# KaffinPX/neptune-core

Measured on AMD Instinct MI355X. Metric: STARK proofs verified/sec (whole node) + Tip5 perms/sec vs VALU roofline, higher is better.
Workload: dtype u64 (Goldilocks mod p; XFE = cubic extension)

## Files before the change

neptune-core_amd/csrc/stark_kernels.hip:

```cpp
#include <hip/hip_ext.h>

#include <atomic>
#include <cstdlib>

#include "../../include/nhip_challenge_id.h"
#include "kernels.hpp"
#include "proof_codec.hpp"
#include "stark.hpp"
#include "tip5_device.hpp"
#include "xfe.hpp"

namespace nhip {

#ifndef NHIP_LAT_PRIO
#define NHIP_LAT_PRIO 2
#endif
__device__ __forceinline__ void latency_priority() {
    if constexpr (NHIP_LAT_PRIO > 0) __builtin_amdgcn_s_setprio(NHIP_LAT_PRIO);
}
static constexpr uint32_t AGE_PRIO_OLDEST = 2;
static constexpr uint32_t AGE_PRIO_MIN_PROOFS = 2048;
__device__ uint32_t g_batches_done;
struct AgePrio {
    uint32_t seq, k;
};
__device__ __forceinline__ void age_priority(AgePrio a, int base) {
    bool old = false;
    if (a.k) {
        const uint32_t done = __builtin_amdgcn_readfirstlane(
            __hip_atomic_load(&g_batches_done, __ATOMIC_RELAXED, __HIP_MEMORY_SCOPE_AGENT));
        old = (int32_t)(a.seq - done) < (int32_t)a.k;
    }
    switch (base + (old ? 1 : 0)) {
        case 0: break;
        case 1: __builtin_amdgcn_s_setprio(1); break;
        case 2: __builtin_amdgcn_s_setprio(2); break;
        default: __builtin_amdgcn_s_setprio(3); break;
    }
}
#ifndef NHIP_MP_PRIO
#define NHIP_MP_PRIO 1
#endif


template <bool MW>
__device__ __forceinline__ Xfe ld_xfe_w(const uint64_t* __restrict__ w, uint64_t off) {
    return {word_mont<MW>(w[off]), word_mont<MW>(w[off + 1]), word_mont<MW>(w[off + 2])};
}
__device__ __forceinline__ Xfe ld_xfe_raw(const uint64_t* __restrict__ w, uint64_t off) {
    return {w[off], w[off + 1], w[off + 2]};
}
__device__ __forceinline__ void st_xfe_raw(uint64_t* __restrict__ w, uint64_t off, Xfe v) {
    w[off] = v.c0;
    w[off + 1] = v.c1;
    w[off + 2] = v.c2;
}
__device__ __forceinline__ bool x_is_zero(Xfe a) { return (a.c0 | a.c1 | a.c2) == 0; }

__device__ __forceinline__ uint64_t root_of_unity(uint32_t log2n) {
    return b_pow(to_mont(7), (GL_P - 1) >> log2n);
}

template <bool MW>
__global__ void __launch_bounds__(64) k_decode(const uint64_t* __restrict__ words, const ProofIn* __restrict__ in,
                                               uint32_t n_proofs, Dims D, uint32_t fs_stride, uint32_t xs_stride,
                                               ProofDesc* __restrict__ desc, FsOp* __restrict__ ops,
                                               uint32_t* __restrict__ fail, unsigned long long* __restrict__ counters) {
    latency_priority();
    __shared__ ProofDesc spd;
    __shared__ uint32_t sfail;
    __shared__ int sdeg;
    const uint32_t p = blockIdx.x, lane = threadIdx.x;
    if (p >= n_proofs) return;
    const ProofIn pin = in[p];
    if (lane == 0) {
        uint64_t perms = 0, perms_lcw = 0;
        const ClaimLoc cl{pin.claim_off, pin.claim_in_n, pin.claim_out_n};
        uint32_t f = decode_stream<MW>(words, pin.off, pin.len, cl, D, spd, ops + (uint64_t)p * fs_stride, perms, perms_lcw);
        if (!f && spd.log2_ph != pin.sized_log2_ph) {
            f = FAIL_DECODE;
            spd = ProofDesc{};
            claim_offsets(spd, cl);
        }
        if (!f) {
            atomicAdd(counters + CNT_PERMS_STATIC, (unsigned long long)perms);
            atomicAdd(counters + CNT_PERMS_LCW, (unsigned long long)perms_lcw);
        }
        sfail = f;
        sdeg = -1;
    }
    __syncthreads();
    const uint32_t f = sfail;
    if (!f) {
        int deg = -1;
        for (uint32_t hi = spd.last_poly_n; hi > 0; hi = hi > 64 ? hi - 64 : 0) {
            bool nz = false;
            if (lane < hi) {
                const uint64_t* x = words + spd.last_poly_off + 3ull * (hi - 1 - lane);
                nz = (canon(x[0]) | canon(x[1]) | canon(x[2])) != 0;
            }
            const uint64_t b = __ballot(nz);
            if (b) {
                deg = (int)(hi - (uint32_t)__ffsll((unsigned long long)b));
                break;
            }
        }
        if (lane == 0) sdeg = deg;
    }
    __syncthreads();
    if (lane == 0) {
        if (!f) last_poly_finish(spd, sdeg, D);
        const SampleLayout sl = SampleLayout::of(D.d, spd.R);
        spd.fs_op_off = p * fs_stride;
        spd.xs_off = (uint64_t)p * xs_stride;
        spd.n_xs = f ? 0u : sl.total;
        spd.idx_off = (uint64_t)p * D.d.num_checks;
        fail[p] = f;
    }
    __syncthreads();
    const uint64_t* src = reinterpret_cast<const uint64_t*>(&spd);
    uint64_t* dst = reinterpret_cast<uint64_t*>(desc + p);
    for (uint32_t i = lane; i < sizeof(ProofDesc) / 8; i += 64) dst[i] = src[i];
}

template <bool PAIR, bool MW>
__device__ __forceinline__ void fs_replay_wide_body(uint32_t bx, const Tip5Lds& lds, const uint64_t* __restrict__ words,
                                                    const ProofDesc* __restrict__ desc,
                                                    const FsOp* __restrict__ ops, uint32_t n_proofs,
                                                    uint64_t* __restrict__ xs, uint32_t* __restrict__ idx_out,
                                                    const uint32_t* __restrict__ fail) {
    constexpr uint32_t LANES = PAIR ? 32u : 16u;
    const uint32_t e = threadIdx.x & 15u;
    const uint32_t h = PAIR ? (threadIdx.x >> 4) & 1u : 0u;
    const uint32_t g = (bx * blockDim.x + threadIdx.x) / LANES;
    if (g >= n_proofs || fail[g]) return;
    uint64_t rc[TIP5_ROUNDS];
#pragma unroll
    for (int r = 0; r < TIP5_ROUNDS; ++r) rc[r] = c_tip5_rc_raw[r * 16 + e];
    uint32_t cm[8];
#pragma unroll
    for (int j = 0; j < 8; ++j) cm[j] = h ? TIP5_MDS[j + 8] : TIP5_MDS[j];
    auto permute = [&](uint64_t st) {
        if constexpr (PAIR) return tip5_permute_pair(st, e, h, rc, cm, lds.lut);
        else return tip5_permute_wide<false>(st, e, rc, lds.lut);
    };
    const bool writer = h == 0;
    const ProofDesc& d = desc[g];
    uint64_t s = 0;
    uint64_t xcur = d.xs_off * 3;
    uint64_t icur = d.idx_off;
    const uint32_t row_shift = threadIdx.x & (64u - LANES);
    for (uint32_t o = 0; o < d.fs_op_n; ++o) {
        const FsOp op = ops[d.fs_op_off + o];
        if (op.kind == FS_ABSORB) {
            const uint64_t* __restrict__ src = words + op.arg;
            const uint32_t len = op.n;
            const uint32_t nchunks = len / TIP5_RATE + 1;
            uint64_t w = (e < TIP5_RATE && e < len) ? src[e] : 0ull;
            for (uint32_t c = 0; c < nchunks; ++c) {
                const uint32_t pos = c * TIP5_RATE;
                const uint64_t cur = w;
                const uint32_t ni = pos + TIP5_RATE + e;
                w = (e < TIP5_RATE && ni < len) ? src[ni] : 0ull;
                if (e < TIP5_RATE) {
                    const uint32_t rem = len - pos;
                    s = e < rem ? word_mont<MW>(cur) : (e == rem ? MONT_ONE : 0ull);
                }
                s = permute(s);
            }
        } else if (op.kind == FS_SQUEEZE_X) {
            const uint32_t nwords = 3 * op.n;
            for (uint32_t f = 0; f < nwords; f += TIP5_RATE) {
                if (writer && e < TIP5_RATE && f + e < nwords) xs[xcur + f + e] = s;
                s = permute(s);
            }
            xcur += nwords;
        } else {
            const uint64_t bound = op.arg;
            uint32_t got = 0;
            while (got < op.n) {
                const uint64_t v = from_mont(s);
                s = permute(s);
                const bool valid = e < TIP5_RATE && v != GL_P - 1;
                const uint64_t ball = __ballot(valid);
                const uint32_t bits = (uint32_t)(ball >> row_shift) & 0x3FFu;
                const uint32_t rank = __popc(bits & ((1u << e) - 1u));
                if (writer && valid && got + rank < op.n) idx_out[icur + got + rank] = (uint32_t)((v & 0xFFFFFFFFull) % bound);
                got += __popc(bits);
            }
            icur += op.n;
        }
    }
}
template <bool PAIR, bool MW>
__global__ void __launch_bounds__(256) k_fs_replay_wide(const uint64_t* __restrict__ words,
                                                        const ProofDesc* __restrict__ desc,
                                                        const FsOp* __restrict__ ops, uint32_t n_proofs,
                                                        uint64_t* __restrict__ xs, uint32_t* __restrict__ idx_out,
                                                        const uint32_t* __restrict__ fail, AgePrio age) {
    age_priority(age, NHIP_LAT_PRIO);
    __shared__ Tip5Lds lds;
    tip5_lds_init(lds);
    fs_replay_wide_body<PAIR, MW>(blockIdx.x, lds, words, desc, ops, n_proofs, xs, idx_out, fail);
}

#ifndef NHIP_QUAD_PRIO
#define NHIP_QUAD_PRIO NHIP_LAT_PRIO
#endif
template <bool MW>
__global__ void __launch_bounds__(1024) k_fs_replay_quad(const uint64_t* __restrict__ words,
                                                       const ProofDesc* __restrict__ desc,
                                                       const FsOp* __restrict__ ops, uint32_t n_proofs,
                                                       uint64_t* __restrict__ xs, uint32_t* __restrict__ idx_out,
// ... 732 lines not shown
        __syncthreads();
    }
}

template <bool MW>
__device__ __forceinline__ void mp_roots_body(uint32_t i, const uint64_t* __restrict__ words,
                                              const ProofDesc* __restrict__ desc, const uint64_t* __restrict__ dig,
                                              MpPlan plan, uint32_t n_records, uint32_t trees_per_proof, uint32_t k,
                                              uint32_t* __restrict__ fail, uint32_t n_proofs, LcwTree lcw) {
    if (i >= n_records) {
        const uint32_t p = i - n_records;
        if (p >= n_proofs || (fail[p] & FAIL_DECODE)) return;
        const ProofDesc& d = desc[p];
        uint64_t v[5];
        lcw_node<MW>(words, d, lcw.nodes + (uint64_t)p * lcw.max_len * 5, 1, d.last_cw_n, v);
        bool ok = true;
#pragma unroll
        for (int q = 0; q < 5; ++q) ok &= v[q] == word_mont<MW>(words[d.fri_root[d.R] + q]);
        if (!ok) atomicOr(&fail[p], FAIL_FRI_LAST_ROOT);
        return;
    }
    const MpRoot r = plan.roots[i];
    if (r.code == MPS_NONE) return;
    const uint32_t p = i / trees_per_proof, tree = i - p * trees_per_proof;
    const ProofDesc& d = desc[p];
    const uint64_t grp_id = (uint64_t)p * (trees_per_proof - 3) + (tree < 4 ? 0u : tree - 3);
    const uint32_t nd = plan.ndup[grp_id];
    bool ok = true;
    for (uint32_t j = 0; j < nd; ++j) {
        uint64_t a[5], b[5];
        mp_load<MW>(mp_leaf_code(d, p, tree, k, plan.dups[(grp_id * k + j) * 2]), words, dig, nullptr, a);
        mp_load<MW>(mp_leaf_code(d, p, tree, k, plan.dups[(grp_id * k + j) * 2 + 1]), words, dig, nullptr, b);
#pragma unroll
        for (int q = 0; q < 5; ++q) ok &= a[q] == b[q];
    }
    uint64_t v[5];
    mp_load<MW>(r.code, words, dig, plan.arena, v);
#pragma unroll
    for (int q = 0; q < 5; ++q) ok &= v[q] == word_mont<MW>(words[r.root_off + q]);
    if (!ok) atomicOr(&fail[p], r.fail_bit);
}
template <bool MW>
__global__ void k_mp_roots(const uint64_t* __restrict__ words, const ProofDesc* __restrict__ desc,
                           const uint64_t* __restrict__ dig, MpPlan plan, uint32_t n_records, uint32_t trees_per_proof,
                           uint32_t k, uint32_t* __restrict__ fail, uint32_t n_proofs, LcwTree lcw) {
    mp_roots_body<MW>(blockIdx.x * blockDim.x + threadIdx.x, words, desc, dig, plan, n_records, trees_per_proof, k,
                      fail, n_proofs, lcw);
}

__device__ Xfe block_sum_xfe(Xfe v, Xfe* sh) {
    const uint32_t tid = threadIdx.x;
    sh[tid] = v;
    __syncthreads();
    for (uint32_t s = blockDim.x >> 1; s > 0; s >>= 1) {
        if (tid < s) sh[tid] = x_add(sh[tid], sh[tid + s]);
        __syncthreads();
    }
    const Xfe r = sh[0];
    __syncthreads();
    return r;
}

__device__ __forceinline__ Xfe shfl_xor_xfe_fwd(Xfe v, int m) {
    return {(uint64_t)__shfl_xor((long long)v.c0, m), (uint64_t)__shfl_xor((long long)v.c1, m),
            (uint64_t)__shfl_xor((long long)v.c2, m)};
}

__device__ Xfe block_sum_xfe_waves(Xfe v, Xfe* sh) {
    const uint32_t tid = threadIdx.x, nw = blockDim.x >> 6;
#pragma unroll
    for (int m = 32; m > 0; m >>= 1) v = x_add(v, shfl_xor_xfe_fwd(v, m));
    if ((tid & 63u) == 0) sh[tid >> 6] = v;
    __syncthreads();
    Xfe r = sh[0];
    for (uint32_t w = 1; w < nw; ++w) r = x_add(r, sh[w]);
    __syncthreads();
    return r;
}

static constexpr uint32_t CH_COMPRESS_PROGRAM_DIGEST = NHIP_CH_CompressProgramDigestIndeterminate,
                          CH_STANDARD_INPUT = NHIP_CH_StandardInputIndeterminate,
                          CH_STANDARD_OUTPUT = NHIP_CH_StandardOutputIndeterminate,
                          CH_LOOKUP_TABLE_PUBLIC = NHIP_CH_LookupTablePublicIndeterminate;
static_assert(CH_LOOKUP_TABLE_PUBLIC == 54 && NHIP_CHALLENGE_SAMPLE_COUNT == 59 && NHIP_CHALLENGE_COUNT == 63,
              "triton-air ChallengeId layout");
static_assert(NHIP_CH_StandardInputTerminal == NHIP_CHALLENGE_SAMPLE_COUNT && NHIP_CH_CompressedProgramDigest == 62,
              "derived challenges follow the sampled ones");

__device__ __forceinline__ Xfe shfl_xor_xfe(Xfe v, int m) {
    return {(uint64_t)__shfl_xor((long long)v.c0, m), (uint64_t)__shfl_xor((long long)v.c1, m),
            (uint64_t)__shfl_xor((long long)v.c2, m)};
}

template <class Sym>
__device__ Xfe eval_terminal_wave(uint32_t n, Xfe c, Sym sym) {
    const uint32_t lane = threadIdx.x & 63u;
    uint32_t s = 0;
    while (s < 6u && (1u << s) < n + 1u) ++s;
    const uint32_t L = 1u << s, ch = (n + L) >> s, pad = L * ch - n;
    auto entry = [&](uint32_t pos) -> Xfe {
        if (lane >= L) return x_zero();
        if (pos >= pad) return x_lift(sym(pos - pad));
        return pos + 1u == pad ? x_one() : x_zero();
    };
    Xfe h = entry(lane * ch), m = c;
    for (uint32_t k = 1; k < ch; ++k) {
        h = x_add(x_mul(h, c), entry(lane * ch + k));
        m = x_mul(m, c);
    }
    for (uint32_t k = 0; k < s; ++k) {
        const Xfe o = shfl_xor_xfe(h, 1 << k);
        const bool up = (lane >> k) & 1u;
        h = x_add(x_mul(up ? o : h, m), up ? h : o);
        if (k + 1u < s) m = x_mul(m, m);
    }
    return h;
}

#ifndef NHIP_OOD_WAVES
#define NHIP_OOD_WAVES 1
#endif

template <uint32_t BLOCK, bool MW, bool GS>
__global__ void __launch_bounds__(BLOCK, BLOCK == 256 ? NHIP_OOD_WAVES : 1) k_ood_air(const uint64_t* __restrict__ words, const ProofDesc* __restrict__ desc,
                                                 uint32_t n_proofs, StarkDims dims, const OodIns* __restrict__ prog,
                                                 const uint32_t* __restrict__ seg_off, uint32_t n_levels,
                                                 const Xfe* __restrict__ consts, uint4 cons_type_off,
                                                 const uint64_t* __restrict__ xs, uint64_t* __restrict__ ood_out,
                                                 uint32_t* __restrict__ fail, uint32_t lds_slots,
                                                 Xfe* __restrict__ gslots, uint32_t gslot_n) {
    latency_priority();
    extern __shared__ __attribute__((aligned(16))) unsigned char smem[];
    Xfe* red = reinterpret_cast<Xfe*>(smem);
    Xfe* zinv = red + 16;
    Xfe* chal_derived = zinv + 4;
    Xfe* misc = chal_derived + 4;
    uint32_t& zero_flag = *reinterpret_cast<uint32_t*>(misc + 4);
    Xfe* val = reinterpret_cast<Xfe*>(smem + AIR_LDS_HEADER);
    const uint32_t p = blockIdx.x, tid = threadIdx.x;
    Xfe* gval = gslots + (uint64_t)p * gslot_n;
    auto slot_ld = [&](uint32_t s) -> Xfe { return !GS || s < lds_slots ? val[s] : gval[s - lds_slots]; };
    auto slot_st = [&](uint32_t s, const Xfe& v) {
        if (!GS || s < lds_slots) val[s] = v;
        else gval[s - lds_slots] = v;
    };
    if (p >= n_proofs || (fail[p] & FAIL_DECODE)) return;
    const ProofDesc& d = desc[p];
    const SampleLayout sl = SampleLayout::of(dims, d.R);
    const uint64_t xb = d.xs_off * 3;
    const Xfe z = ld_xfe_raw(xs, xb + 3ull * sl.z);
    if (tid == 0) zero_flag = 0;
    __syncthreads();
    if (tid == 0) {
        const uint64_t w_inv = b_inv(root_of_unity(d.log2_ph));
        const Xfe except_last = x_sub(z, x_lift(w_inv));
        const Xfe zm1 = x_sub(z, x_one());
        Xfe zph = z;
        for (uint32_t q = 0; q < d.log2_ph; ++q) zph = x_mul(zph, zph);
        const Xfe cons = x_sub(zph, x_one());
        const bool z0 = x_is_zero(zm1), z1 = x_is_zero(cons), z3 = x_is_zero(except_last);
        if (z0 || z1 || z3) zero_flag = 1u;
        const Xfe a = z0 ? x_one() : zm1, b = z1 ? x_one() : cons, c = z3 ? x_one() : except_last;
        const Xfe ab = x_mul(a, b);
        const Xfe iabc = x_inv(x_mul(ab, c));
        const Xfe iab = x_mul(iabc, c);
        const Xfe i1 = z1 ? x_zero() : x_mul(iab, a);
        zinv[0] = z0 ? x_zero() : x_mul(iab, b);
        zinv[1] = i1;
        zinv[2] = x_mul(except_last, i1);
        zinv[3] = z3 ? x_zero() : x_mul(iabc, ab);
    } else if (tid >= 64 && tid < 256) {
        auto chal = [&](uint32_t i) { return ld_xfe_raw(xs, xb + 3ull * (sl.chal + i)); };
        const uint32_t wv = tid >> 6;
        if (wv == 1) {
            const Xfe lut = eval_terminal_wave(256u, chal(CH_LOOKUP_TABLE_PUBLIC), [&](uint32_t i) {
                const uint64_t y = i + 1;
                return to_mont((y * y % 257u * y % 257u + 256u) % 257u);
            });
            if (tid == 64) chal_derived[2] = lut;
        } else if (wv == 2) {
            const Xfe ein = eval_terminal_wave(d.claim_in_n, chal(CH_STANDARD_INPUT),
                                               [&](uint32_t i) { return word_mont<MW>(words[d.claim_in_off + i]); });
            const Xfe comp = eval_terminal_wave(5u, chal(CH_COMPRESS_PROGRAM_DIGEST),
                                                [&](uint32_t i) { return word_mont<MW>(words[d.claim_digest_off + i]); });
            if (tid == 128) {
                chal_derived[0] = ein;
                chal_derived[3] = comp;
            }
        } else {
            const Xfe eout = eval_terminal_wave(d.claim_out_n, chal(CH_STANDARD_OUTPUT),
                                                [&](uint32_t i) { return word_mont<MW>(words[d.claim_out_off + i]); });
            if (tid == 192) chal_derived[1] = eout;
        }
    }
    __syncthreads();
    const uint32_t offs[5] = {0u, cons_type_off.x, cons_type_off.y, cons_type_off.z, cons_type_off.w};
    auto fetch = [&](uint32_t ref) -> Xfe {
        const uint32_t t = ref >> 30;
        if (t == 0) return slot_ld(ref);
        if (t == 1) return consts[ref & 0x3FFFFFFFu];
        const uint32_t kind = (ref >> 27) & 7u, i = ref & 0x7FFFFFFu;
        switch (kind) {
            case IN_MAIN_CURR: return ld_xfe_w<MW>(words, d.ood_mc + 3ull * i);
            case IN_AUX_CURR: return ld_xfe_w<MW>(words, d.ood_ac + 3ull * i);
            case IN_MAIN_NEXT: return ld_xfe_w<MW>(words, d.ood_mn + 3ull * i);
            case IN_AUX_NEXT: return ld_xfe_w<MW>(words, d.ood_an + 3ull * i);
            default:
                return i < dims.num_sampled ? ld_xfe_raw(xs, xb + 3ull * (sl.chal + i)) : chal_derived[i - dims.num_sampled];
        }
    };
    for (uint32_t lvl = 0; lvl < n_levels; ++lvl) {
        const uint32_t s0 = seg_off[3 * lvl], s1 = seg_off[3 * lvl + 1], s2 = seg_off[3 * lvl + 2],
                       s3 = seg_off[3 * lvl + 3];
        for (uint32_t q = s0 + tid; q < s1; q += blockDim.x) {
            const uint4 ins = reinterpret_cast<const uint4*>(prog)[q];
            slot_st(ins.w, fetch(ins.y));
        }
        for (uint32_t q = s1 + tid; q < s2; q += blockDim.x) {
            const uint4 ins = reinterpret_cast<const uint4*>(prog)[q];
            slot_st(ins.w, x_mul(slot_ld(ins.y), slot_ld(ins.z)));
        }
        for (uint32_t q = s2 + tid; q < s3; q += blockDim.x) {
            const uint4 ins = reinterpret_cast<const uint4*>(prog)[q];
            const Xfe x = slot_ld(ins.y), y = slot_ld(ins.z);
            slot_st(ins.w, ins.x == OOD_ADD ? x_add(x, y) : x_sub(x, y));
        }
        __syncthreads();
    }
    const uint32_t C = dims.num_constraints, cbase = lds_slots + gslot_n - C;
    Xfe acc = x_zero();
    for (uint32_t c = tid; c < C; c += blockDim.x) {
        uint32_t t = 0;
        while (t < 3 && c >= offs[t + 1]) ++t;
        const Xfe w = ld_xfe_raw(xs, xb + 3ull * (sl.quot_w + c));
        acc = x_add(acc, x_mul(w, x_mul(slot_ld(cbase + c), zinv[t])));
    }
    const Xfe ood_q = block_sum_xfe_waves(acc, red);
    const uint32_t M = dims.num_main, A = dims.num_aux, Q = dims.num_quot_seg;
    Xfe lc = x_zero(), ln = x_zero();
    for (uint32_t c = tid; c < M + A; c += blockDim.x) {
        const Xfe w = ld_xfe_raw(xs, xb + 3ull * (sl.lin_w + c));
        const Xfe vc = c < M ? ld_xfe_w<MW>(words, d.ood_mc + 3ull * c) : ld_xfe_w<MW>(words, d.ood_ac + 3ull * (c - M));
        const Xfe vn = c < M ? ld_xfe_w<MW>(words, d.ood_mn + 3ull * c) : ld_xfe_w<MW>(words, d.ood_an + 3ull * (c - M));
        lc = x_add(lc, x_mul(w, vc));
        ln = x_add(ln, x_mul(w, vn));
    }
    const Xfe sum_c = block_sum_xfe_waves(lc, red);
    const Xfe sum_n = block_sum_xfe_waves(ln, red);
    if (tid >= 64) return;
    Xfe seg = x_zero(), qlin = x_zero();
    for (uint32_t base = 0; base < Q; base += 64u) {
        const uint32_t q = base + tid, top = min(Q - 1u, base + 63u);
        Xfe zk = (q & 1u) ? z : x_one(), zp = z;
        for (uint32_t e = top >> 1, bit = 1; e; e >>= 1, ++bit) {
            zp = x_mul(zp, zp);
            zk = x_mul(zk, ((q >> bit) & 1u) ? zp : x_one());
        }
        if (q < Q) {
            const Xfe sq = ld_xfe_w<MW>(words, d.ood_qs + 3ull * q);
            seg = x_add(seg, x_mul(zk, sq));
            qlin = x_add(qlin, x_mul(ld_xfe_raw(xs, xb + 3ull * (sl.lin_w + M + A + q)), sq));
        }
    }
#pragma unroll
    for (int m = 32; m > 0; m >>= 1) {
        seg = x_add(seg, shfl_xor_xfe(seg, m));
        qlin = x_add(qlin, shfl_xor_xfe(qlin, m));
    }
    if (tid == 0) {
        uint32_t f = 0;
        if (zero_flag) f |= FAIL_ZERO_INVERSE;
        if (!x_eq(seg, ood_q)) f |= FAIL_OOD;
        if (f) atomicOr(&fail[p], f);
        uint64_t* o = ood_out + (uint64_t)p * 9;
        st_xfe_raw(o, 0, sum_c);
        st_xfe_raw(o, 3, sum_n);
        st_xfe_raw(o, 6, qlin);
    }
}

__device__ __forceinline__ uint64_t lds_pow(const uint64_t* __restrict__ sq, uint64_t e) {
    uint64_t r = MONT_ONE;
    for (uint32_t b = 0; e; ++b, e >>= 1)
        if (e & 1) r = mont_mul(r, sq[b]);
    return r;
}

#ifndef NHIP_FRI_WAVES
#define NHIP_FRI_WAVES 1
#endif
template <bool MW>
__device__ __forceinline__ void fri_body(uint32_t p, const uint64_t* __restrict__ words, const ProofDesc* __restrict__ desc,
                                         uint32_t n_proofs, StarkDims dims, const uint64_t* __restrict__ xs,
                                         const uint32_t* __restrict__ idx_all, uint64_t* __restrict__ xdom,
                                         uint32_t* __restrict__ fail) {
    __shared__ Xfe red[256];
    __shared__ uint64_t gsq[33], wsq[33];
    __shared__ uint32_t lflag;
    const uint32_t tid = threadIdx.x;
    if (p >= n_proofs || (fail[p] & FAIL_DECODE)) return;
    const ProofDesc& d = desc[p];
    const SampleLayout sl = SampleLayout::of(dims, d.R);
    const uint64_t xb = d.xs_off * 3;
    const uint32_t k = dims.num_checks;
    const uint32_t* __restrict__ idx = idx_all + d.idx_off;
    const uint32_t L = d.last_cw_n;
    const uint32_t log2L = 31 - __clz(L);
    if (tid == 0) {
        lflag = 0;
        uint64_t g = root_of_unity(d.log2_N);
        for (uint32_t q = 0; q < d.log2_N; ++q, g = mont_mul(g, g)) gsq[q] = g;
    } else if (tid == 64) {
        uint64_t w = root_of_unity(log2L);
        for (uint32_t q = 0; q < log2L; ++q, w = mont_mul(w, w)) wsq[q] = w;
    }
    __syncthreads();
    uint32_t f = 0;
    if (tid < k) {
        const uint32_t i0 = idx[tid];
        Xfe a = ld_xfe_w<MW>(words, d.fri[0].leaves_off + 3ull * tid);
        uint64_t x = mont_mul(to_mont(7), lds_pow(gsq, i0));
        xdom[(uint64_t)p * k + tid] = x;
        uint64_t xinv = b_inv(x);
        const uint64_t neg_half = to_mont((GL_P - 1) / 2);
        for (uint32_t r = 0; r < d.R; ++r) {
            const Xfe b = ld_xfe_w<MW>(words, d.fri[1 + r].leaves_off + 3ull * tid);
            const Xfe alpha = ld_xfe_raw(xs, xb + 3ull * (sl.alpha + r));
            const Xfe slope = x_scale(x_sub(b, a), mont_mul(neg_half, xinv));
            a = x_add(a, x_mul(slope, x_sub(alpha, x_lift(x))));
            x = mont_mul(x, x);
            xinv = mont_mul(xinv, xinv);
        }
        const Xfe last = ld_xfe_w<MW>(words, d.last_cw_off + 3ull * (i0 & (L - 1)));
        if (!x_eq(last, a)) f |= FAIL_FRI_LAST_AGREE;
    }
    const Xfe t = ld_xfe_raw(xs, xb + 3ull * sl.indeterminate);
    Xfe num = x_zero(), den = x_zero();
    if (tid < L) {
        uint64_t wi = lds_pow(wsq, tid);
        const uint64_t wstep = blockDim.x < L ? wsq[31 - __clz(blockDim.x)] : MONT_ONE;
        auto term = [&](uint32_t i, uint64_t w, Xfe inv) {
            const Xfe q = x_scale(inv, w);
            num = x_add(num, x_mul(q, ld_xfe_w<MW>(words, d.last_cw_off + 3ull * i)));
            den = x_add(den, q);
        };
        uint32_t i = tid;
        for (; i + blockDim.x < L; i += 2 * blockDim.x) {
            const uint64_t w1 = mont_mul(wi, wstep);
            const Xfe d0 = x_sub(t, x_lift(wi)), d1 = x_sub(t, x_lift(w1));
            const Xfe pr = x_mul(d0, d1);
            if (x_is_zero(pr)) {
                atomicOr(&lflag, 1u);
                term(i, wi, x_inv(d0));
                term(i + blockDim.x, w1, x_inv(d1));
            } else {
                const Xfe inv = x_inv(pr);
                term(i, wi, x_mul(inv, d1));
                term(i + blockDim.x, w1, x_mul(inv, d0));
            }
            wi = mont_mul(w1, wstep);
        }
        if (i < L) {
            const Xfe diff = x_sub(t, x_lift(wi));
            if (x_is_zero(diff)) atomicOr(&lflag, 1u);
            term(i, wi, x_inv(diff));
        }
    }
    const Xfe snum = block_sum_xfe(num, red);
    const Xfe sden = block_sum_xfe(den, red);
    __shared__ Xfe tpow[32];
    const uint32_t pbits = d.last_poly_n ? 32 - __clz(d.last_poly_n) : 0;
    if (tid == 0) {
        Xfe q = t;
        for (uint32_t j = 0; j < pbits; ++j, q = x_mul(q, q)) tpow[j] = q;
    }
    __syncthreads();
    Xfe hp = x_zero();
    for (uint32_t c = tid; c < d.last_poly_n; c += blockDim.x) {
        Xfe pw = x_one();
        for (uint32_t j = 0; (c >> j) != 0; ++j)
            if ((c >> j) & 1u) pw = x_mul(pw, tpow[j]);
        hp = x_add(hp, x_mul(pw, ld_xfe_w<MW>(words, d.last_poly_off + 3ull * c)));
    }
    const Xfe h = block_sum_xfe(hp, red);
    if (tid == 0) {
        if (lflag || x_is_zero(sden)) f |= FAIL_ZERO_INVERSE;
        else if (!x_eq(h, x_mul(snum, x_inv(sden)))) f |= FAIL_FRI_EVAL;
        if (!d.last_poly_degree_ok) f |= FAIL_FRI_DEGREE;
    }
    if (f) atomicOr(&fail[p], f);
}
template <bool MW>
__global__ void __launch_bounds__(256, NHIP_FRI_WAVES) k_fri(const uint64_t* __restrict__ words, const ProofDesc* __restrict__ desc,
                                             uint32_t n_proofs, StarkDims dims, const uint64_t* __restrict__ xs,
                                             const uint32_t* __restrict__ idx_all, uint64_t* __restrict__ xdom,
                                             uint32_t* __restrict__ fail) {
    latency_priority();
    fri_body<MW>(blockIdx.x, words, desc, n_proofs, dims, xs, idx_all, xdom, fail);
}

template <bool MW>
__global__ void __launch_bounds__(256) k_plan_fri_small(const uint64_t* __restrict__ words,
                                                        const ProofDesc* __restrict__ desc, uint32_t n_proofs,
                                                        uint32_t k, uint32_t trees_per_proof, uint32_t groups,
                                                        const uint64_t* __restrict__ dig,
                                                        const uint32_t* __restrict__ idx_all, MpPlan plan,
                                                        uint32_t* __restrict__ fail,
                                                        unsigned long long* __restrict__ perm_counter,
                                                        StarkDims dims, const uint64_t* __restrict__ xs,
                                                        uint64_t* __restrict__ xdom) {
    latency_priority();
    const uint32_t bx = blockIdx.x, np = n_proofs * groups;
    if (bx < np)
        mp_plan_body<256>(bx % n_proofs, bx / n_proofs, words, desc, n_proofs, k, trees_per_proof, dig, idx_all, plan,
                          fail, perm_counter);
    else
        fri_body<MW>(bx - np, words, desc, n_proofs, dims, xs, idx_all, xdom, fail);
}

typedef unsigned __int128 u128_t;
static constexpr uint32_t DEEP_UNROLL = 8;

__device__ __forceinline__ uint64_t reduce_u108(u128_t y) {
    const uint64_t y0 = (uint64_t)y, y1 = (uint64_t)(y >> 64);
    const uint64_t r = reduce96(y0, (uint32_t)y1);
    return gl_sub(r, y1 >> 32);
}

__device__ __forceinline__ uint64_t shfl_xor_u64(uint64_t v, int m) {
    return (uint64_t)__shfl_xor((long long)v, m);
}

__device__ __forceinline__ uint4 w_limbs(uint64_t w) {
    return make_uint4((uint32_t)w & 0x3FFFFFu, (uint32_t)(w >> 22) & 0x3FFFFFu, (uint32_t)(w >> 44), 0u);
}
__device__ __forceinline__ void wl_mac(uint64_t (&a)[6], uint4 wl, uint32_t x0, uint32_t x1) {
    a[0] += (uint64_t)wl.x * x0;
    a[1] += (uint64_t)wl.y * x0;
    a[2] += (uint64_t)wl.z * x0;
    a[3] += (uint64_t)wl.x * x1;
    a[4] += (uint64_t)wl.y * x1;
    a[5] += (uint64_t)wl.z * x1;
}
__device__ __forceinline__ uint64_t wl_reduce(const uint64_t (&a)[6]) {
    const u128_t U = (u128_t)a[0] + ((u128_t)a[1] << 22) + ((u128_t)a[2] << 44);
    const u128_t W = (u128_t)a[3] + ((u128_t)a[4] << 22) + ((u128_t)a[5] << 44);
    const uint64_t ur = reduce_u108(U), wr = reduce_u108(W);
    return gl_add(ur, reduce96(wr << 32, (uint32_t)(wr >> 32)));
}

#ifndef NHIP_DEEP_WAVES
#define NHIP_DEEP_WAVES 6
#endif
template <bool MW>
__global__ void __launch_bounds__(256, NHIP_DEEP_WAVES) k_deep_rows8(const uint64_t* __restrict__ words,
                                                    const ProofDesc* __restrict__ desc, uint32_t n_proofs,
                                                    StarkDims dims, const uint64_t* __restrict__ xs,
                                                    const uint64_t* __restrict__ xdom,
                                                    const uint64_t* __restrict__ ood, uint32_t* __restrict__ fail) {
    extern __shared__ __attribute__((aligned(16))) unsigned char smem[];
    const uint32_t M = dims.num_main, A = dims.num_aux, Q = dims.num_quot_seg, k = dims.num_checks;
    uint4* wm = reinterpret_cast<uint4*>(smem);
    uint4* wa = wm + 3 * M;
    Xfe* rowsum = reinterpret_cast<Xfe*>(wa + 9 * A);
    __shared__ Xfe s_quot[MAX_CHECKS];
    __shared__ Xfe s_at[3];
    const uint32_t p = blockIdx.x, tid = threadIdx.x;
    if (p >= n_proofs || (fail[p] & FAIL_DECODE)) return;
    const ProofDesc& d = desc[p];
    const SampleLayout sl = SampleLayout::of(dims, d.R);
    const uint64_t xb = d.xs_off * 3;
    const uint64_t* __restrict__ lw = xs + xb + 3ull * sl.lin_w;
    for (uint32_t i = tid; i < 3 * M; i += blockDim.x) wm[i] = w_limbs(lw[i]);
    for (uint32_t c = tid; c < A; c += blockDim.x) {
        const uint64_t w0 = lw[3 * (M + c)], w1 = lw[3 * (M + c) + 1], w2 = lw[3 * (M + c) + 2];
        uint4* o = wa + 9 * c;
        o[0] = w_limbs(w0), o[1] = w_limbs(w1), o[2] = w_limbs(w2);
        o[3] = w_limbs(gl_sub(0, w2)), o[4] = w_limbs(gl_add(w0, w2)), o[5] = w_limbs(w1);
        o[6] = w_limbs(gl_sub(0, w1)), o[7] = w_limbs(gl_sub(w1, w2)), o[8] = w_limbs(gl_add(w0, w2));
    }
    if (tid == blockDim.x - 1) {
        const Xfe z = ld_xfe_raw(xs, xb + 3ull * sl.z);
        s_at[0] = z;
        s_at[1] = x_scale(z, root_of_unity(d.log2_ph));
        Xfe zq = x_one();
        for (uint32_t q = 0; q < Q; ++q) zq = x_mul(zq, z);
        s_at[2] = zq;
    }
    __syncthreads();
    const uint32_t q8 = tid & 7u, rloc = tid >> 3;
    const uint32_t rows_per_pass = blockDim.x >> 3;
    for (uint32_t j0 = 0; j0 < k; j0 += rows_per_pass) {
        const uint32_t j = j0 + rloc;
        uint64_t acc[3][6];
#pragma unroll
        for (int c = 0; c < 3; ++c)
#pragma unroll
            for (int q = 0; q < 6; ++q) acc[c][q] = 0;
        if (j < k) {
            const uint64_t* __restrict__ mrow = words + d.main_rows_off + (uint64_t)j * M;
            uint32_t c = q8;
            for (; c + 8 * (DEEP_UNROLL - 1) < M; c += 8 * DEEP_UNROLL) {
                uint64_t xv[DEEP_UNROLL];
#pragma unroll
                for (uint32_t u = 0; u < DEEP_UNROLL; ++u) xv[u] = mrow[c + 8 * u];
#pragma unroll
                for (uint32_t u = 0; u < DEEP_UNROLL; ++u) {
                    const uint32_t cc = c + 8 * u, x0 = (uint32_t)xv[u], x1 = (uint32_t)(xv[u] >> 32);
                    wl_mac(acc[0], wm[3 * cc], x0, x1);
                    wl_mac(acc[1], wm[3 * cc + 1], x0, x1);
                    wl_mac(acc[2], wm[3 * cc + 2], x0, x1);
                }
            }
            for (; c < M; c += 8) {
                const uint64_t xw = mrow[c];
                const uint32_t x0 = (uint32_t)xw, x1 = (uint32_t)(xw >> 32);
                wl_mac(acc[0], wm[3 * c], x0, x1);
                wl_mac(acc[1], wm[3 * c + 1], x0, x1);
                wl_mac(acc[2], wm[3 * c + 2], x0, x1);
            }
            const uint64_t* __restrict__ arow = words + d.aux_rows_off + (uint64_t)j * 3 * A;
            const uint32_t WA = 3 * A;
            uint32_t w = q8;
            for (; w + 8 * (DEEP_UNROLL - 1) < WA; w += 8 * DEEP_UNROLL) {
                uint64_t xv[DEEP_UNROLL];
#pragma unroll
                for (uint32_t u = 0; u < DEEP_UNROLL; ++u) xv[u] = arow[w + 8 * u];
#pragma unroll
                for (uint32_t u = 0; u < DEEP_UNROLL; ++u) {
                    const uint4* wt = wa + 3 * (w + 8 * u);
                    const uint32_t x0 = (uint32_t)xv[u], x1 = (uint32_t)(xv[u] >> 32);
                    wl_mac(acc[0], wt[0], x0, x1);
                    wl_mac(acc[1], wt[1], x0, x1);
                    wl_mac(acc[2], wt[2], x0, x1);
                }
            }
            for (; w < WA; w += 8) {
                const uint4* wt = wa + 3 * w;
                const uint64_t xw = arow[w];
                const uint32_t x0 = (uint32_t)xw, x1 = (uint32_t)(xw >> 32);
                wl_mac(acc[0], wt[0], x0, x1);
                wl_mac(acc[1], wt[1], x0, x1);
                wl_mac(acc[2], wt[2], x0, x1);
            }
        }
        uint64_t v0 = wl_reduce(acc[0]), v1 = wl_reduce(acc[1]), v2 = wl_reduce(acc[2]);
#pragma unroll
        for (int m = 1; m < 8; m <<= 1) {
            v0 = gl_add(v0, shfl_xor_u64(v0, m));
            v1 = gl_add(v1, shfl_xor_u64(v1, m));
            v2 = gl_add(v2, shfl_xor_u64(v2, m));
        }
        if (j < k && q8 == 0) {
            if constexpr (MW) rowsum[j] = {from_mont(v0), from_mont(v1), from_mont(v2)};
            else rowsum[j] = {v0, v1, v2};
        }
        if (j < k && q8 == 1) {
            Xfe qv = x_zero();
            for (uint32_t q = 0; q < Q; ++q)
                qv = x_add(qv, x_mul(ld_xfe_raw(lw, 3ull * (M + A + q)),
                                     ld_xfe_raw(words, d.quot_rows_off + (uint64_t)j * 3 * Q + 3ull * q)));
            if constexpr (MW) s_quot[j] = qv;
            else s_quot[j] = {to_mont(qv.c0), to_mont(qv.c1), to_mont(qv.c2)};
        }
    }
    __syncthreads();
    uint32_t f = 0;
    for (uint32_t j2 = tid; j2 < k; j2 += blockDim.x) {
        const Xfe row = rowsum[j2];
        const Xfe x = x_lift(xdom[(uint64_t)p * k + j2]);
        const Xfe d0 = x_sub(x, s_at[0]), d1 = x_sub(x, s_at[1]), d2 = x_sub(x, s_at[2]);
        const Xfe d01 = x_mul(d0, d1);
        const Xfe prod = x_mul(d01, d2);
        if (x_is_zero(prod)) {
            f |= FAIL_ZERO_INVERSE;
            continue;
        }
        const Xfe inv = x_inv(prod);
        const Xfe inv2 = x_mul(inv, d01);
        const Xfe inv01 = x_mul(inv, d2);
        const Xfe inv0 = x_mul(inv01, d1);
        const Xfe inv1 = x_mul(inv01, d0);
        const uint64_t* __restrict__ oo = ood + (uint64_t)p * 9;
        const uint64_t* __restrict__ wd = lw + 3ull * (M + A + Q);
        const Xfe t0 = x_mul(x_mul(x_sub(row, ld_xfe_raw(oo, 0)), inv0), ld_xfe_raw(wd, 0));
        const Xfe t1 = x_mul(x_mul(x_sub(row, ld_xfe_raw(oo, 3)), inv1), ld_xfe_raw(wd, 3));
        const Xfe t2 = x_mul(x_mul(x_sub(s_quot[j2], ld_xfe_raw(oo, 6)), inv2), ld_xfe_raw(wd, 6));
        const Xfe deep = x_add(x_add(t0, t1), t2);
        const Xfe fri_v = ld_xfe_w<MW>(words, d.fri[0].leaves_off + 3ull * j2);
        if (!x_eq(deep, fri_v)) f |= FAIL_DEEP;
    }
    if (f) atomicOr(&fail[p], f);
}

__global__ void k_verdicts(const uint32_t* __restrict__ fail, uint32_t n, uint8_t* __restrict__ v) {
    const uint32_t i = blockIdx.x * blockDim.x + threadIdx.x;
    if (i < n) v[i] = fail[i] == 0 ? 1 : 0;
    if (i == 0) atomicAdd(&g_batches_done, 1u);
}
static constexpr uint32_t ROOTS_ONE_WG = 1024;
template <bool MW>
__global__ void __launch_bounds__(ROOTS_ONE_WG) k_roots_verdicts_small(
    const uint64_t* __restrict__ words, const ProofDesc* __restrict__ desc, const uint64_t* __restrict__ dig,
    MpPlan plan, uint32_t n_records, uint32_t trees_per_proof, uint32_t k, uint32_t* __restrict__ fail,
    uint32_t n_proofs, LcwTree lcw, uint8_t* __restrict__ v) {
    const uint32_t i = threadIdx.x;
    mp_roots_body<MW>(i, words, desc, dig, plan, n_records, trees_per_proof, k, fail, n_proofs, lcw);
    __threadfence();
    __syncthreads();
    if (i < n_proofs) v[i] = __hip_atomic_load(&fail[i], __ATOMIC_RELAXED, __HIP_MEMORY_SCOPE_AGENT) == 0 ? 1 : 0;
    if (i == 0) atomicAdd(&g_batches_done, 1u);
}

template <typename K, typename... A>
static void launch_ev(K kernel, dim3 grid, dim3 block, size_t shm, hipStream_t s, hipEvent_t e0, hipEvent_t e1,
                      A... args) {
    if (e0 || e1) hipExtLaunchKernelGGL(kernel, grid, block, shm, s, e0, e1, 0, args...);
    else hipLaunchKernelGGL(kernel, grid, block, shm, s, args...);
}

static bool ood_wide(uint32_t n) {
    static const uint32_t lim = [] {
        const char* v = nhip::ab_env("NHIP_OOD_WIDE_MAX");
        return v ? (uint32_t)std::strtoul(v, nullptr, 10) : OOD_WIDE_MAX_PROOFS;
    }();
    return n <= lim;
}

static constexpr uint32_t CLIMB_FROM_MIN_LEVELS = 24;
static constexpr uint64_t CLIMB_FROM_OPS_DEFAULT = 4096;
static std::atomic<int64_t>& climb_from_forced() {
    static std::atomic<int64_t> v(-1);
    return v;
}
int set_climb_from_ops(int64_t ops) {
    if (ops < -1) return -1;
    climb_from_forced().store(ops, std::memory_order_relaxed);
    return 0;
}
static uint64_t climb_from_ops(uint32_t hash_levels) {
    const int64_t v = climb_from_forced().load(std::memory_order_relaxed);
    if (v >= 0) return (uint64_t)v;
    return hash_levels >= CLIMB_FROM_MIN_LEVELS ? CLIMB_FROM_OPS_DEFAULT : 0ull;
}


static constexpr uint32_t ROWS_WIDE_MAX_PROOFS = 32;
static uint32_t rows_wide_max() {
    static const uint32_t v = [] {
        const char* e = nhip::ab_env("NHIP_ROWS_WIDE_MAX");
        return e ? (uint32_t)std::strtoul(e, nullptr, 10) : ROWS_WIDE_MAX_PROOFS;
    }();
    return v;
}

enum FsForm { FS_ROW = 0, FS_PAIR = 1, FS_QUAD = 2 };
static uint32_t quad_wg() {
    static const uint32_t v = [] {
        const char* e = nhip::ab_env("NHIP_QUAD_WG");
        const uint32_t w = e ? (uint32_t)std::strtoul(e, nullptr, 10) : FS_QUAD_WG;
        return (w >= 64 && w <= 1024 && w % 64 == 0) ? w : FS_QUAD_WG;
    }();
    return v;
}
static std::atomic<int>& fs_form_forced() {
    static std::atomic<int> f([] {
        if (const char* v = nhip::ab_env("NHIP_FS_FORM")) {
            if (v[0] == 'q') return (int)FS_QUAD;
            if (v[0] == 'p') return (int)FS_PAIR;
            if (v[0] == 'r') return (int)FS_ROW;
        }
        return -1;
    }());
    return f;
}
int set_fs_form(int form) {
    if (form < -1 || form > (int)FS_QUAD) return -1;
    fs_form_forced().store(form, std::memory_order_relaxed);
    return 0;
}
static FsForm fs_form(uint32_t n) {
    static const uint32_t quad_min = [] {
        const char* v = nhip::ab_env("NHIP_FS_QUAD_MIN");
        return v ? (uint32_t)std::strtoul(v, nullptr, 10) : FS_QUAD_MIN_PROOFS;
    }();
    const int forced = fs_form_forced().load(std::memory_order_relaxed);
    if (forced >= 0) return (FsForm)forced;
    if (n < FS_PAIR_MAX_PROOFS) return FS_PAIR;
    return n >= quad_min ? FS_QUAD : FS_ROW;
}

#ifdef NHIP_AB_BUILD
__global__ void k_pad_packet() {}
#endif

template <bool MW>
static hipError_t launch_phases(const StarkBatchDev& b, hipStream_t st, hipStream_t sa, StarkPhaseTimer* tm) {
    const uint32_t n = b.n_proofs;
    if (n == 0) return hipSuccess;
    (void)hipGetLastError();
    const uint32_t k = b.dims.num_checks;
    const uint32_t tpp = 4 + b.max_R;
    const bool two = st != sa;
    constexpr uint32_t SYNC = (1u << 12) | (1u << 0) | (1u << 1) | (1u << 3) | (1u << 7) | (1u << 10) | (1u << 8);
    auto mark = [&](int i, hipStream_t s) {
        if (tm->phase_marks || (two && ((SYNC >> i) & 1u))) (void)hipEventRecord(tm->ev[i], s);
    };
    auto wait = [&](hipStream_t s, int i) {
        if (two) (void)hipStreamWaitEvent(s, tm->ev[i], 0);
    };
#ifdef NHIP_AB_BUILD
    static const int pad_n = [] {
        const char* e = nhip::ab_env("NHIP_PAD_PACKETS");
        return e ? std::atoi(e) : 0;
    }();
    auto pad = [&](hipStream_t s) {
// ... 232 lines not shown
```

neptune-core_amd/csrc/xfe.hpp:

```cpp
#pragma once
#include "goldilocks.hpp"

namespace nhip {

struct Xfe {
    uint64_t c0, c1, c2;
};

static constexpr uint64_t MONT_ONE_W = 0x00000000FFFFFFFFull;

__host__ __device__ __forceinline__ Xfe x_zero() { return {0, 0, 0}; }
__host__ __device__ __forceinline__ Xfe x_one() { return {MONT_ONE_W, 0, 0}; }
__host__ __device__ __forceinline__ Xfe x_lift(uint64_t b) { return {b, 0, 0}; }

__host__ __device__ __forceinline__ Xfe x_add(Xfe a, Xfe b) {
    return {gl_add(a.c0, b.c0), gl_add(a.c1, b.c1), gl_add(a.c2, b.c2)};
}
__host__ __device__ __forceinline__ Xfe x_sub(Xfe a, Xfe b) {
    return {gl_sub(a.c0, b.c0), gl_sub(a.c1, b.c1), gl_sub(a.c2, b.c2)};
}
__host__ __device__ __forceinline__ Xfe x_scale(Xfe a, uint64_t s) {
    return {mont_mul(a.c0, s), mont_mul(a.c1, s), mont_mul(a.c2, s)};
}
__host__ __device__ __forceinline__ bool x_eq(Xfe a, Xfe b) { return a.c0 == b.c0 && a.c1 == b.c1 && a.c2 == b.c2; }

struct U128 {
    uint64_t lo, hi;
};
struct U160 {
    uint64_t lo, hi;
    uint32_t top;
};

__host__ __device__ __forceinline__ U128 mul128(uint64_t a, uint64_t b) {
    const uint32_t a0 = (uint32_t)a, a1 = (uint32_t)(a >> 32);
    const uint32_t b0 = (uint32_t)b, b1 = (uint32_t)(b >> 32);
    const uint64_t p00 = (uint64_t)a0 * b0;
    const uint64_t t = (uint64_t)a0 * b1 + (p00 >> 32);
    const uint64_t u = (uint64_t)a1 * b0 + (uint32_t)t;
    const uint64_t v = (uint64_t)a1 * b1 + (t >> 32);
    return {(u << 32) | (uint32_t)p00, v + (u >> 32)};
}

__host__ __device__ __forceinline__ U160 add160(U160 x, U128 y) {
    unsigned int c0, c1, c2, c3;
    const uint32_t l0 = __builtin_addc((uint32_t)x.lo, (uint32_t)y.lo, 0u, &c0);
    const uint32_t l1 = __builtin_addc((uint32_t)(x.lo >> 32), (uint32_t)(y.lo >> 32), c0, &c1);
    const uint32_t h0 = __builtin_addc((uint32_t)x.hi, (uint32_t)y.hi, c1, &c2);
    const uint32_t h1 = __builtin_addc((uint32_t)(x.hi >> 32), (uint32_t)(y.hi >> 32), c2, &c3);
    return {((uint64_t)l1 << 32) | l0, ((uint64_t)h1 << 32) | h0, x.top + c3};
}
__host__ __device__ __forceinline__ U160 wide(U128 x) { return {x.lo, x.hi, 0u}; }

__host__ __device__ __forceinline__ U160 sub160_2p(U160 x, U160 y) {
    unsigned int c0, c1, b0, b1, b2, b3;
    const uint32_t h0 = __builtin_addc((uint32_t)x.hi, 2u, 0u, &c0);
    const uint32_t h1 = __builtin_addc((uint32_t)(x.hi >> 32), 0xFFFFFFFEu, c0, &c1);
    const uint32_t l0 = __builtin_subc((uint32_t)x.lo, (uint32_t)y.lo, 0u, &b0);
    const uint32_t l1 = __builtin_subc((uint32_t)(x.lo >> 32), (uint32_t)(y.lo >> 32), b0, &b1);
    const uint32_t g0 = __builtin_subc(h0, (uint32_t)y.hi, b1, &b2);
    const uint32_t g1 = __builtin_subc(h1, (uint32_t)(y.hi >> 32), b2, &b3);
    return {((uint64_t)l1 << 32) | l0, ((uint64_t)g1 << 32) | g0, x.top + 1u + c1 - y.top - b3};
}

__host__ __device__ __forceinline__ uint64_t red160(U160 x) {
    const uint64_t tt = ((uint64_t)x.top << 32) - x.top;
    uint64_t h = x.hi + tt;
    if (h < tt) h += GL_EPS;
    const uint32_t xl0 = (uint32_t)x.lo, xl1 = (uint32_t)(x.lo >> 32);
    unsigned int e, br1, br2, c1, c, c2;
    const uint32_t ah = __builtin_addc(xl1, xl0, 0u, &e);
    const uint32_t bl = __builtin_subc(xl0, ah, e, &br1);
    const uint32_t bh = __builtin_subc(ah, 0u, br1, &br2);
    uint32_t rl = __builtin_subc((uint32_t)h, bl, 0u, &c1);
    uint32_t rh = __builtin_subc((uint32_t)(h >> 32), bh, c1, &c);
    const uint32_t m = 0u - c;
    rl = __builtin_subc(rl, m, 0u, &c2);
    rh = rh - c2;
    const uint64_t r = ((uint64_t)rh << 32) | rl;
    return r >= GL_P ? r - GL_P : r;
}

__host__ __device__ __forceinline__ Xfe x_mul(Xfe a, Xfe b) {
    const U128 p12 = mul128(a.c1, b.c2), p21 = mul128(a.c2, b.c1), p00 = mul128(a.c0, b.c0);
    const U160 n = add160(wide(p12), p21);
    Xfe r;
    r.c0 = red160(sub160_2p(wide(p00), n));
    const U128 p01 = mul128(a.c0, b.c1), p10 = mul128(a.c1, b.c0), p22 = mul128(a.c2, b.c2);
    U160 s1 = add160(add160(wide(p01), p10), U128{n.lo, n.hi});
    s1.top += n.top;
    r.c1 = red160(sub160_2p(s1, wide(p22)));
    const U128 p02 = mul128(a.c0, b.c2), p11 = mul128(a.c1, b.c1), p20 = mul128(a.c2, b.c0);
    r.c2 = red160(add160(add160(add160(wide(p02), p11), p20), p22));
    return r;
}

__host__ __device__ __forceinline__ uint64_t b_sqn(uint64_t x, int n) {
#pragma unroll 1
    for (int i = 0; i < n; ++i) x = mont_mul(x, x);
    return x;
}

__host__ __device__ __forceinline__ uint64_t b_inv(uint64_t a) {
    const uint64_t t2 = mont_mul(mont_mul(a, a), a);
    const uint64_t t3 = mont_mul(mont_mul(t2, t2), a);
    const uint64_t t6 = mont_mul(b_sqn(t3, 3), t3);
    const uint64_t t12 = mont_mul(b_sqn(t6, 6), t6);
    const uint64_t t15 = mont_mul(b_sqn(t12, 3), t3);
    const uint64_t t30 = mont_mul(b_sqn(t15, 15), t15);
    const uint64_t t31 = mont_mul(mont_mul(t30, t30), a);
    const uint64_t t32m2 = mont_mul(t31, t31);
    const uint64_t t32 = mont_mul(t32m2, a);
    return mont_mul(b_sqn(t32m2, 32), t32);
}

__host__ __device__ __forceinline__ uint64_t b_pow(uint64_t a, uint64_t e) {
    uint64_t r = MONT_ONE_W;
    while (e) {
        if (e & 1) r = mont_mul(r, a);
        a = mont_mul(a, a);
        e >>= 1;
    }
    return r;
}

__host__ __device__ __forceinline__ Xfe x_inv(Xfe a) {
    const uint64_t s = gl_add(a.c0, a.c2);
    const uint64_t d = gl_sub(a.c1, a.c2);
    const uint64_t C00 = gl_sub(mont_mul(s, s), mont_mul(d, a.c1));
    const uint64_t C01 = gl_sub(mont_mul(d, a.c2), mont_mul(a.c1, s));
    const uint64_t C02 = gl_sub(mont_mul(a.c1, a.c1), mont_mul(s, a.c2));
    const uint64_t det = gl_sub(gl_sub(mont_mul(a.c0, C00), mont_mul(a.c2, C01)), mont_mul(a.c1, C02));
    const uint64_t di = b_inv(det);
    return {mont_mul(C00, di), mont_mul(C01, di), mont_mul(C02, di)};
}

__host__ __device__ __forceinline__ Xfe x_pow(Xfe a, uint64_t e) {
    Xfe r = x_one();
    while (e) {
        if (e & 1) r = x_mul(r, a);
        a = x_mul(a, a);
        e >>= 1;
    }
    return r;
}

}
```

Baseline: 467,900.

## Precompute two-adic roots, avoid inversions in FRI, batch barycentric inverses per lane

Roots of unity and their inverses become constexpr tables, so per-block b_pow and b_inv calls are gone. The FRI domain inverse is now computed as 7^-1 times g^(-i), which removes a per-query field inversion. The last-codeword barycentric evaluation uses Montgomery batch inversion across up to 8 points per lane, with strided point assignment, and a parallel table fill replaces the serial squaring loops. The quotient-row combination moves out of a branch taken by a single lane group into a strided loop over all threads. The risks are more register and stack use from the per-lane arrays, and correctness depends on the zero-handling in the batched slot.

```diff
diff --git a/neptune-core_amd/csrc/stark_kernels.hip b/neptune-core_amd/csrc/stark_kernels.hip
--- a/neptune-core_amd/csrc/stark_kernels.hip
+++ b/neptune-core_amd/csrc/stark_kernels.hip
@@ -54,11 +54,6 @@
     w[off] = v.c0;
     w[off + 1] = v.c1;
     w[off + 2] = v.c2;
-}
-__device__ __forceinline__ bool x_is_zero(Xfe a) { return (a.c0 | a.c1 | a.c2) == 0; }
-
-__device__ __forceinline__ uint64_t root_of_unity(uint32_t log2n) {
-    return b_pow(to_mont(7), (GL_P - 1) >> log2n);
 }
 
 template <bool MW>
@@ -1097,7 +1092,7 @@
     if (tid == 0) zero_flag = 0;
     __syncthreads();
     if (tid == 0) {
-        const uint64_t w_inv = b_inv(root_of_unity(d.log2_ph));
+        const uint64_t w_inv = root_of_unity_inv(d.log2_ph);
         const Xfe except_last = x_sub(z, x_lift(w_inv));
         const Xfe zm1 = x_sub(z, x_one());
         Xfe zph = z;
@@ -1224,12 +1219,6 @@
     }
 }
 
-__device__ __forceinline__ uint64_t lds_pow(const uint64_t* __restrict__ sq, uint64_t e) {
-    uint64_t r = MONT_ONE;
-    for (uint32_t b = 0; e; ++b, e >>= 1)
-        if (e & 1) r = mont_mul(r, sq[b]);
-    return r;
-}
 
 #ifndef NHIP_FRI_WAVES
 #define NHIP_FRI_WAVES 1
@@ -1251,14 +1240,9 @@
     const uint32_t* __restrict__ idx = idx_all + d.idx_off;
     const uint32_t L = d.last_cw_n;
     const uint32_t log2L = 31 - __clz(L);
-    if (tid == 0) {
-        lflag = 0;
-        uint64_t g = root_of_unity(d.log2_N);
-        for (uint32_t q = 0; q < d.log2_N; ++q, g = mont_mul(g, g)) gsq[q] = g;
-    } else if (tid == 64) {
-        uint64_t w = root_of_unity(log2L);
-        for (uint32_t q = 0; q < log2L; ++q, w = mont_mul(w, w)) wsq[q] = w;
-    }
+    if (tid == 0) lflag = 0;
+    if (tid < d.log2_N && tid < 33) gsq[tid] = root_of_unity(d.log2_N - tid);
+    if (tid < log2L) wsq[tid] = root_of_unity(log2L - tid);
     __syncthreads();
     uint32_t f = 0;
     if (tid < k) {
@@ -1266,7 +1250,7 @@
         Xfe a = ld_xfe_w<MW>(words, d.fri[0].leaves_off + 3ull * tid);
         uint64_t x = mont_mul(to_mont(7), lds_pow(gsq, i0));
         xdom[(uint64_t)p * k + tid] = x;
-        uint64_t xinv = b_inv(x);
+        uint64_t xinv = mont_mul(SEVEN_INV, lds_pow(gsq, neg_mod_pow2(i0, d.log2_N)));
         const uint64_t neg_half = to_mont((GL_P - 1) / 2);
         for (uint32_t r = 0; r < d.R; ++r) {
             const Xfe b = ld_xfe_w<MW>(words, d.fri[1 + r].leaves_off + 3ull * tid);
@@ -1281,35 +1265,12 @@
     }
     const Xfe t = ld_xfe_raw(xs, xb + 3ull * sl.indeterminate);
     Xfe num = x_zero(), den = x_zero();
-    if (tid < L) {
-        uint64_t wi = lds_pow(wsq, tid);
-        const uint64_t wstep = blockDim.x < L ? wsq[31 - __clz(blockDim.x)] : MONT_ONE;
-        auto term = [&](uint32_t i, uint64_t w, Xfe inv) {
-            const Xfe q = x_scale(inv, w);
-            num = x_add(num, x_mul(q, ld_xfe_w<MW>(words, d.last_cw_off + 3ull * i)));
-            den = x_add(den, q);
-        };
-        uint32_t i = tid;
-        for (; i + blockDim.x < L; i += 2 * blockDim.x) {
-            const uint64_t w1 = mont_mul(wi, wstep);
-            const Xfe d0 = x_sub(t, x_lift(wi)), d1 = x_sub(t, x_lift(w1));
-            const Xfe pr = x_mul(d0, d1);
-            if (x_is_zero(pr)) {
-                atomicOr(&lflag, 1u);
-                term(i, wi, x_inv(d0));
-                term(i + blockDim.x, w1, x_inv(d1));
-            } else {
-                const Xfe inv = x_inv(pr);
-                term(i, wi, x_mul(inv, d1));
-                term(i + blockDim.x, w1, x_mul(inv, d0));
-            }
-            wi = mont_mul(w1, wstep);
-        }
-        if (i < L) {
-            const Xfe diff = x_sub(t, x_lift(wi));
-            if (x_is_zero(diff)) atomicOr(&lflag, 1u);
-            term(i, wi, x_inv(diff));
-        }
+    {
+        const uint32_t ppl = bary_points_per_lane(L), S = (L + ppl - 1) / ppl;
+        const uint64_t wS = root_of_unity(31 - __clz(ppl));
+        auto cw = [&](uint32_t i) { return ld_xfe_w<MW>(words, d.last_cw_off + 3ull * i); };
+        for (uint32_t s = blockDim.x - 1 - tid; s < S; s += blockDim.x)
+            if (bary_slot(t, lds_pow(wsq, s), wS, s, S, L, ppl, cw, num, den)) atomicOr(&lflag, 1u);
     }
     const Xfe snum = block_sum_xfe(num, red);
     const Xfe sden = block_sum_xfe(den, red);
@@ -1424,6 +1385,14 @@
         o[3] = w_limbs(gl_sub(0, w2)), o[4] = w_limbs(gl_add(w0, w2)), o[5] = w_limbs(w1);
         o[6] = w_limbs(gl_sub(0, w1)), o[7] = w_limbs(gl_sub(w1, w2)), o[8] = w_limbs(gl_add(w0, w2));
     }
+    for (uint32_t j = tid; j < k; j += blockDim.x) {
+        Xfe qv = x_zero();
+        for (uint32_t q = 0; q < Q; ++q)
+            qv = x_add(qv, x_mul(ld_xfe_raw(lw, 3ull * (M + A + q)),
+                                 ld_xfe_raw(words, d.quot_rows_off + (uint64_t)j * 3 * Q + 3ull * q)));
+        if constexpr (MW) s_quot[j] = qv;
+        else s_quot[j] = {to_mont(qv.c0), to_mont(qv.c1), to_mont(qv.c2)};
+    }
     if (tid == blockDim.x - 1) {
         const Xfe z = ld_xfe_raw(xs, xb + 3ull * sl.z);
         s_at[0] = z;
@@ -1499,14 +1468,6 @@
         if (j < k && q8 == 0) {
             if constexpr (MW) rowsum[j] = {from_mont(v0), from_mont(v1), from_mont(v2)};
             else rowsum[j] = {v0, v1, v2};
-        }
-        if (j < k && q8 == 1) {
-            Xfe qv = x_zero();
-            for (uint32_t q = 0; q < Q; ++q)
-                qv = x_add(qv, x_mul(ld_xfe_raw(lw, 3ull * (M + A + q)),
-                                     ld_xfe_raw(words, d.quot_rows_off + (uint64_t)j * 3 * Q + 3ull * q)));
-            if constexpr (MW) s_quot[j] = qv;
-            else s_quot[j] = {to_mont(qv.c0), to_mont(qv.c1), to_mont(qv.c2)};
         }
     }
     __syncthreads();
diff --git a/neptune-core_amd/csrc/xfe.hpp b/neptune-core_amd/csrc/xfe.hpp
--- a/neptune-core_amd/csrc/xfe.hpp
+++ b/neptune-core_amd/csrc/xfe.hpp
@@ -124,6 +124,44 @@
     return r;
 }
 
+namespace two_adic {
+constexpr uint64_t mulp(uint64_t a, uint64_t b) { return (uint64_t)(((unsigned __int128)a * b) % GL_P); }
+constexpr uint64_t powp(uint64_t a, uint64_t e) {
+    uint64_t r = 1;
+    for (; e; e >>= 1, a = mulp(a, a))
+        if (e & 1) r = mulp(r, a);
+    return r;
+}
+constexpr uint64_t raw(uint64_t x) { return (uint64_t)(((unsigned __int128)x << 64) % GL_P); }
+struct Roots {
+    uint64_t root[33], inv[33];
+};
+constexpr Roots make() {
+    Roots t{};
+    for (int k = 0; k <= 32; ++k) {
+        const uint64_t r = powp(7, (GL_P - 1) >> k);
+        t.root[k] = raw(r);
+        t.inv[k] = raw(powp(r, GL_P - 2));
+    }
+    return t;
+}
+}
+static constexpr two_adic::Roots TWO_ADIC_ROOTS = two_adic::make();
+static constexpr uint64_t SEVEN_INV = two_adic::raw(two_adic::powp(7, GL_P - 2));
+
+__host__ __device__ __forceinline__ uint64_t root_of_unity(uint32_t log2n) { return TWO_ADIC_ROOTS.root[log2n]; }
+__host__ __device__ __forceinline__ uint64_t root_of_unity_inv(uint32_t log2n) { return TWO_ADIC_ROOTS.inv[log2n]; }
+
+__host__ __device__ __forceinline__ uint64_t lds_pow(const uint64_t* __restrict__ sq, uint64_t e) {
+    uint64_t r = MONT_ONE_W;
+    for (uint32_t b = 0; e; ++b, e >>= 1)
+        if (e & 1) r = mont_mul(r, sq[b]);
+    return r;
+}
+__host__ __device__ __forceinline__ uint32_t neg_mod_pow2(uint32_t i, uint32_t log2_N) {
+    return (0u - i) & (log2_N >= 32 ? ~0u : (1u << log2_N) - 1u);
+}
+
 __host__ __device__ __forceinline__ Xfe x_inv(Xfe a) {
     const uint64_t s = gl_add(a.c0, a.c2);
     const uint64_t d = gl_sub(a.c1, a.c2);
@@ -145,4 +183,43 @@
     return r;
 }
 
-}
+__host__ __device__ __forceinline__ bool x_is_zero(Xfe a) { return (a.c0 | a.c1 | a.c2) == 0; }
+
+static constexpr uint32_t BARY_PPL_MAX = 8;
+__host__ __device__ __forceinline__ uint32_t bary_points_per_lane(uint32_t L) {
+    uint32_t ppl = 1;
+    while (ppl < BARY_PPL_MAX && (L + ppl - 1) / ppl > 64) ppl *= 2;
+    return ppl;
+}
+template <typename Cw>
+__host__ __device__ __forceinline__ bool bary_slot(Xfe t, uint64_t w0, uint64_t wS, uint32_t s, uint32_t S, uint32_t L,
+                                                   uint32_t ppl, Cw cw, Xfe& num, Xfe& den) {
+    uint64_t wv[BARY_PPL_MAX];
+    Xfe pre[BARY_PPL_MAX];
+    bool zero = false;
+    Xfe acc = x_one();
+    uint64_t w = w0;
+    uint32_t n = 0;
+#pragma unroll 1
+    for (; n < ppl && n < BARY_PPL_MAX && s + (uint64_t)n * S < L; ++n) {
+        Xfe df = x_sub(t, x_lift(w));
+        if (x_is_zero(df)) zero = true, df = x_one();
+        wv[n] = w;
+        pre[n] = acc;
+        acc = n ? x_mul(acc, df) : df;
+        w = mont_mul(w, wS);
+    }
+    Xfe inv = x_inv(acc);
+#pragma unroll 1
+    for (uint32_t j = n; j-- > 0;) {
+        Xfe df = x_sub(t, x_lift(wv[j]));
+        if (x_is_zero(df)) df = x_one();
+        const Xfe q = x_scale(j ? x_mul(inv, pre[j]) : inv, wv[j]);
+        if (j) inv = x_mul(inv, df);
+        num = x_add(num, x_mul(q, cw(s + j * S)));
+        den = x_add(den, q);
+    }
+    return zero;
+}
+
+}
```

Result: faster. 472,800, median of 6 (+1.1%).
